# shehryar-malik/icrl

Measured on NVIDIA B200. Metric: learner transitions/sec per ICRL iteration at 1/2/4/8 B200 vs host CPU, higher is better.
Workload: dtype f32

## Files before the change

### icrl_b200/_lib.py

```python
import ctypes as C
import os

HERE = os.path.dirname(os.path.abspath(__file__))
LIB_PATH = os.path.join(HERE, "libicrl_b200.so")

ABI_VERSION = 2
MAX_SELECT, MAX_HIDDEN, CN_MAX_WIDTH = 512, 3, 64
PPO_STATS_PER_STEP = 8

c_float_p = C.POINTER(C.c_float)
c_void = C.c_void_p


class CnDesc(C.Structure):
    _fields_ = [
        ("obs_dim", C.c_int32), ("acs_dim", C.c_int32), ("is_discrete", C.c_int32), ("n_select", C.c_int32),
        ("select", C.c_int32 * MAX_SELECT), ("n_hidden", C.c_int32), ("hidden", C.c_int32 * MAX_HIDDEN),
        ("has_norm", C.c_int32), ("has_clip_obs", C.c_int32), ("has_clip_acs", C.c_int32), ("clip_obs", C.c_double),
        ("params", c_void), ("obs_mean", c_void), ("obs_rstd", c_void), ("acs_low", c_void), ("acs_high", c_void),
    ]


class CnTrainCfg(C.Structure):
    _fields_ = [
        ("iterations", C.c_int32), ("importance_sampling", C.c_int32), ("per_step_is", C.c_int32),
        ("train_gail_lambda", C.c_int32), ("eps", C.c_float), ("regularizer_coeff", C.c_float),
        ("target_kl_old_new", C.c_float), ("target_kl_new_old", C.c_float), ("lr", C.c_double),
        ("adam_beta1", C.c_double), ("adam_beta2", C.c_double), ("adam_eps", C.c_double),
        ("batch_size", C.c_int32), ("perm", c_void),
    ]

# ... 41 lines not shown

SIGNATURES = {
    "icrl_abi_version": (C.c_int, []),
    "icrl_last_error": (C.c_char_p, []),
    "icrl_launch_count": (C.c_int64, []),
    "icrl_device_info": (C.c_int, [C.POINTER(C.c_int32), C.POINTER(C.c_int32)]),
    "icrl_measure_peaks": (C.c_int, [C.POINTER(C.c_double), c_void]),
    "icrl_cn_param_count": (C.c_int64, [C.POINTER(CnDesc)]),
    "icrl_cn_forward": (C.c_int, [C.POINTER(CnDesc), c_void, C.c_int32, c_void, C.c_int64, c_void, C.c_int32, c_void]),
    "icrl_cn_forward_host": (C.c_int, [C.POINTER(CnDesc), c_void, C.c_int32, c_void, C.c_int64, c_void, C.c_int32,
                                       c_void]),
    "icrl_cn_train": (C.c_int, [C.POINTER(CnDesc), C.POINTER(CnTrainCfg), c_void, C.c_int32, c_void, C.c_int64, c_void,
                                C.c_int32, c_void, C.c_int32, c_void, C.c_int64, c_void, c_void, C.POINTER(C.c_int64),
                                C.POINTER(CnTrainMetrics), c_void]),
    "icrl_cn_dist_bytes": (C.c_int64, [C.POINTER(CnDesc), C.c_int32]),
    "icrl_cn_train_dist": (C.c_int, [C.POINTER(CnDesc), C.POINTER(CnTrainCfg), c_void, C.c_int32, c_void, C.c_int64, c_void,
                                     C.c_int32, c_void, C.c_int32, c_void, C.c_int64, c_void, c_void, C.POINTER(C.c_int64),
                                     C.POINTER(CnTrainMetrics), C.POINTER(CnDist), c_void]),
    "icrl_dual_gae": (C.c_int, [c_void] * 8 + [C.c_int32, C.c_int32] + [C.c_double] * 4 + [c_void] * 5),
    "icrl_dual_gae_host": (C.c_int, [c_void] * 8 + [C.c_int32, C.c_int32] + [C.c_double] * 4 + [c_void] * 5),
    "icrl_ppo_param_count": (C.c_int64, [C.POINTER(PpoCfg)]),
    "icrl_ppo_train": (C.c_int, [C.POINTER(PpoCfg), C.POINTER(PpoData), c_void, c_void, c_void, C.c_int64, c_void,
                                 c_void, c_void]),
    "icrl_ppo_train_dist": (C.c_int, [C.POINTER(PpoCfg), C.POINTER(PpoData), c_void, c_void, c_void, C.c_int64, c_void,
                                      c_void, C.POINTER(PpoDist), c_void]),
    "icrl_ppo_local_advsums": (C.c_int, [C.POINTER(PpoCfg), C.POINTER(PpoData), c_void, c_void]),
    "icrl_comm_alloc": (C.c_int, [C.c_int64, C.POINTER(c_void), C.c_char_p]),
    "icrl_comm_open": (C.c_int, [C.c_char_p, C.POINTER(c_void)]),
    "icrl_comm_close": (C.c_int, [c_void]),
    "icrl_comm_free": (C.c_int, [c_void]),
    "icrl_policy_forward": (C.c_int, [C.POINTER(PpoCfg), c_void, c_void, C.c_int64, c_void, c_void, c_void, c_void]),
    "icrl_dual_update": (C.c_int, [c_void, c_void, C.c_int64, C.c_double, C.c_double, C.c_int64, C.c_double, c_void]),
    "icrl_cost_normalize": (C.c_int, [c_void, c_void, c_void, C.c_int32, C.c_int32, C.c_double, C.c_double, C.c_double,
                                      C.c_int32, C.c_int32, c_void, c_void, c_void]),
}


class IcrlError(RuntimeError):
    pass


_lib = None


def lib():
    global _lib
# ... 32 lines not shown
```

### icrl_b200/csrc/k4_common.cuh

```cuda
#pragma once
#include <math.h>
#include <stdlib.h>

#include "common.cuh"

namespace icrl {

constexpr int H = 64;
constexpr int RB = 64;
constexpr int NTH = 256;
constexpr int AMAX = 16;
constexpr int WA_LD = 68;
constexpr int LDH = 68;
constexpr float LOG_SQRT_2PI = 0.91893853320467274178f;
constexpr float HALF_LOG_2PI_PLUS_HALF = 1.4189385332046727418f;

__host__ __device__ inline int ppo_kp(int D) { return (D + 7) / 8 * 8; }
__host__ __device__ inline int ppo_ldx(int D) {
    const int kp = (D + 15) / 16 * 16;
    int ld = kp / 32 * 32 + 4;
    if (ld < kp) ld += 32;
    return ld;
}

// ... 50 lines not shown
    }
    return o;
}

inline int ppo_make_args(const icrl_ppo_cfg* c, PpoArgs& a) {
    ICRL_CHECK_ARG(c != nullptr, "ppo cfg is NULL");
    ICRL_CHECK_ARG(c->obs_dim >= 1, "obs_dim must be >= 1");
    ICRL_CHECK_ARG(c->act_dim >= 1 && c->act_dim <= AMAX, "act_dim %d out of range (1..%d)", c->act_dim, AMAX);
    bool per_trunk = false;
    for (int t = 0; t < 3; ++t) per_trunk |= c->trunk_hidden[t][0] != 0 || c->trunk_hidden[t][1] != 0;
    if (per_trunk) {
        static const char* const names[3] = {"pi", "vf", "cvf"};
        for (int t = 0; t < 3; ++t)
            ICRL_CHECK_ARG(c->trunk_hidden[t][0] >= 1 && c->trunk_hidden[t][0] <= H && c->trunk_hidden[t][1] >= 1 &&
                               c->trunk_hidden[t][1] <= H,
                           "trunk_hidden[%d] (%s) = (%d, %d): both widths must be in 1..%d (two hidden layers per trunk)", t,
                           names[t], c->trunk_hidden[t][0], c->trunk_hidden[t][1], H);
    } else {
        ICRL_CHECK_ARG(c->hidden[0] >= 1 && c->hidden[0] <= H && c->hidden[1] >= 1 && c->hidden[1] <= H,
                       "policy hidden sizes (%d, %d) must be in 1..%d (two hidden layers per trunk)", c->hidden[0],
                       c->hidden[1], H);
    }
    a.D = c->obs_dim; a.DP = ppo_ldx(c->obs_dim); a.KP = ppo_kp(c->obs_dim); a.A = c->act_dim; a.is_discrete = c->is_discrete;
    for (int t = 0; t < 3; ++t) {
        a.h0[t] = per_trunk ? c->trunk_hidden[t][0] : c->hidden[0];
        a.h1[t] = per_trunk ? c->trunk_hidden[t][1] : c->hidden[1];
    }
    a.T = c->T; a.E = c->E; a.N = c->T * c->E;
    a.B = c->batch_size > 0 ? c->batch_size : a.N;
    if (a.B > a.N && a.N > 0) a.B = a.N;
    a.n_epochs = c->n_epochs;
    a.steps_per_epoch = a.N > 0 ? (a.N + a.B - 1) / a.B : 0;
    a.max_steps = c->max_steps;
    a.has_target_kl = c->has_target_kl; a.has_clip_vf_r = c->has_clip_vf_reward; a.has_clip_vf_c = c->has_clip_vf_cost;
    a.clip_range = c->clip_range; a.clip_vf_r = c->clip_range_reward_vf; a.clip_vf_c = c->clip_range_cost_vf;
    a.ent_coef = c->ent_coef; a.vf_coef_r = c->reward_vf_coef; a.vf_coef_c = c->cost_vf_coef;
    a.max_grad_norm = c->max_grad_norm; a.nu = c->nu; a.target_kl = c->target_kl;
    a.lr = c->lr; a.beta1 = c->adam_beta1; a.beta2 = c->adam_beta2; a.adam_eps = c->adam_eps;
    ppo_fill_offsets(a);
    return 0;
}

}
```

### icrl_b200/csrc/k4_ppo_lag.cu

```cuda
#include <type_traits>

#include "k4_common.cuh"

namespace icrl {

__device__ __forceinline__ uint32_t cluster_ctarank() {
    uint32_t r;
    asm volatile("mov.u32 %0, %%cluster_ctarank;" : "=r"(r));
    return r;
}
__device__ __forceinline__ uint32_t cluster_nctarank() {
    uint32_t r;
    asm volatile("mov.u32 %0, %%cluster_nctarank;" : "=r"(r));
    return r;
}
__device__ __forceinline__ void cluster_sync_all() {
    asm volatile("barrier.cluster.arrive.release.aligned;\n\tbarrier.cluster.wait.acquire.aligned;" ::: "memory");
}
__device__ __forceinline__ void st_remote_f32(float* local_ptr, uint32_t rank, float v) {
    uint32_t a = smem_u32(local_ptr), ra;
    asm volatile("mapa.shared::cluster.u32 %0, %1, %2;" : "=r"(ra) : "r"(a), "r"(rank));
    asm volatile("st.shared::cluster.f32 [%0], %1;" ::"r"(ra), "f"(v) : "memory");
}

// ... 1465 lines not shown
    for (int e = 0; e < n_epochs; ++e) {
        a.n_epochs = 1;
        a.epoch_base = e;
        a.perm = perm + (size_t)e * a.N;
        a.stats = stats + (size_t)e * spe * ICRL_PPO_STATS_PER_STEP;
        a.advsums = advsums ? advsums + (size_t)e * spe * 4 : nullptr;
        a.step_before = step_before + (long long)e * spe;
        a.flag_base = flag_base + (unsigned int)(e * spe);
        ppo_gather_kernel<<<ggrid, 256, 0, st>>>(a, xs, as, ss, (long long)a.N, n_alloc);
        ICRL_LAUNCH_CHECK();
        ppo_stats_kernel<<<spe, 128, 0, st>>>(ss, advstats, a.N, a.B, spe, a.beta1, a.beta2, a.lr, a.step_before, a.advsums);
        ICRL_LAUNCH_CHECK();
        ICRL_CUDA(cudaMemsetAsync(sync, 0, 64, st));
        const cudaError_t err = cudaLaunchKernelEx(&cfg, kern, a);
        if (err != cudaSuccess) {
            set_error("wide ppo_train_kernel launch failed: %s", cudaGetErrorString(err));
            return (int)err;
        }
        count_launch();
    }
    return 0;
}

}

extern "C" {

int64_t icrl_ppo_param_count(const icrl_ppo_cfg* cfg) {
    icrl::PpoArgs a = {};
    if (icrl::ppo_make_args(cfg, a)) return -1;
    return icrl::ppo_fill_offsets(a);
}

static void ppo_print_timing(unsigned long long* timing_dev, cudaStream_t st, double steps);

static int ppo_train_impl(const icrl_ppo_cfg* cfg, const icrl_ppo_data* data, float* params, float* adam_m, float* adam_v,
                          int64_t adam_step_before, float* step_stats, int32_t* result, const icrl_ppo_dist* dist,
                          void* stream) {
    icrl::PpoArgs a = {};
    int rc = icrl::ppo_make_args(cfg, a);
    if (rc) return rc;
    if (dist) {
        ICRL_CHECK_ARG(dist->world >= 1 && dist->world <= ICRL_PPO_MAX_RANKS && dist->rank >= 0 && dist->rank < dist->world,
                       "bad rank/world (%d/%d)", dist->rank, dist->world);
        a.rank = dist->rank; a.world = dist->world; a.flag_base = dist->flag_base; a.advsums = dist->advsums;
        for (int r = 0; r < dist->world; ++r) {
            ICRL_CHECK_ARG(dist->world == 1 || (dist->recv[r] && dist->flags[r]), "peer buffer %d is NULL", r);
            a.recv[r] = dist->recv[r]; a.flags[r] = dist->flags[r];
        }
        ICRL_CHECK_ARG(dist->world == 1 || dist->advsums, "data-parallel mode needs the all-reduced advsums table");
    }
    ICRL_CHECK_ARG(data && params && adam_m && adam_v && step_stats && result, "NULL pointer passed to icrl_ppo_train");
    ICRL_CHECK_ARG(a.N > 0 && a.n_epochs > 0, "empty rollout buffer or n_epochs <= 0");
    ICRL_CHECK_ARG(data->observations && data->actions && data->old_log_prob && data->reward_advantages &&
                       data->reward_returns && data->cost_advantages && data->cost_returns && data->perm,
                   "NULL rollout array");
    ICRL_CHECK_ARG((!a.has_clip_vf_r || data->old_reward_values) && (!a.has_clip_vf_c || data->old_cost_values),
                   "value clipping enabled but old values are NULL");
    a.obs = data->observations; a.act = data->actions; a.old_logp = data->old_log_prob;
    a.old_vr = data->old_reward_values ? data->old_reward_values : data->reward_returns;
    a.adv_r = data->reward_advantages; a.ret_r = data->reward_returns;
    a.old_vc = data->old_cost_values ? data->old_cost_values : data->cost_returns;
    a.adv_c = data->cost_advantages; a.ret_c = data->cost_returns;
    a.perm = data->perm;
    a.nu_dev = data->nu_device;
    a.params = params; a.adam_m = adam_m; a.adam_v = adam_v; a.stats = step_stats; a.result = result;
    a.step_before = adam_step_before;
    if (a.world < 1) { a.world = 1; a.rank = 0; }
    {
        const char* m = getenv("ICRL_PPO_DIST_MODE");
        a.dist_mode = m ? atoi(m) : 0;
    }
    cudaStream_t st = (cudaStream_t)stream;
    ICRL_CUDA(cudaMemsetAsync(result, 0, 4 * sizeof(int32_t), st));
    const int n_tiles = a.KP / 8;
    const int nt1 = (n_tiles + 1) / 2;
    if (nt1 > 8) {
        icrl::set_error("obs_dim %d too large for the PPO kernel (max 128)", a.D);
        return ICRL_EUNSUPPORTED;
    }
    static unsigned long long* timing_dev = nullptr;
    const bool want_timing = getenv("ICRL_PPO_TIMING") != nullptr;
    if (want_timing && !timing_dev) cudaMalloc(&timing_dev, 128 * sizeof(unsigned long long));
    a.timing = want_timing ? timing_dev : nullptr;
    auto print_timing = [&](double steps) { ppo_print_timing(timing_dev, st, steps); };
    bool wide = a.B >= icrl::WIDE_MIN_BATCH;
    if (const char* m = getenv("ICRL_PPO_WIDE")) wide = atoi(m) != 0;
    int n_clusters = 1;
    if (wide) {
        int cap = 0;
        if (nt1 <= 1) rc = icrl::wide_max_clusters<1>(a, st, &cap);
        else if (nt1 <= 2) rc = icrl::wide_max_clusters<2>(a, st, &cap);
        else if (nt1 <= 4) rc = icrl::wide_max_clusters<4>(a, st, &cap);
        else rc = icrl::wide_max_clusters<8>(a, st, &cap);
        if (rc) return rc;
        if (cap > icrl::WIDE_MAXCTA / icrl::NCTA) cap = icrl::WIDE_MAXCTA / icrl::NCTA;
        const int useful = (a.B + icrl::RB - 1) / icrl::RB;
        n_clusters = cap < useful ? cap : useful;
        if (const char* m = getenv("ICRL_PPO_WIDE_CLUSTERS")) {
            const int c = atoi(m);
            if (c > 0) n_clusters = c < cap ? c : cap;
        }
        const int nt1r = nt1 <= 1 ? 1 : nt1 <= 2 ? 2 : nt1 <= 4 ? 4 : 8;
        const int F = icrl::NTW2 * 4 + nt1r * 4 + 4 + 1 + 5;
        if (n_clusters < 1 || 2 * n_clusters * icrl::WIDE_SMAX < F) wide = false;
    }
    {
        const int epochs_alloc = wide ? 1 : a.n_epochs;
        const int total_steps = epochs_alloc * a.steps_per_epoch;
        const long long n_rows = (long long)epochs_alloc * a.N, n_alloc = n_rows + icrl::RB;
        const int aw = a.is_discrete ? 1 : a.A;
        a.AP = (aw + 3) / 4 * 4;
        void *xs, *as, *ss, *advstats;
        if ((rc = icrl::device_scratch(icrl::SLOT_PPO0, (size_t)n_alloc * a.DP * 4, &xs))) return rc;
        if ((rc = icrl::device_scratch(icrl::SLOT_PPO1, (size_t)total_steps * 8 * sizeof(float), &advstats))) return rc;
        if ((rc = icrl::device_scratch(icrl::SLOT_PPO2, (size_t)n_alloc * a.AP * 4, &as))) return rc;
        if ((rc = icrl::device_scratch(icrl::SLOT_PPO3, (size_t)n_alloc * 8 * 4, &ss))) return rc;
        if (wide) {
            if (nt1 <= 1) rc = icrl::launch_ppo_wide<1>(a, st, n_clusters, (float*)xs, (float*)as, (float*)ss, (float*)advstats);
            else if (nt1 <= 2) rc = icrl::launch_ppo_wide<2>(a, st, n_clusters, (float*)xs, (float*)as, (float*)ss, (float*)advstats);
            else if (nt1 <= 4) rc = icrl::launch_ppo_wide<4>(a, st, n_clusters, (float*)xs, (float*)as, (float*)ss, (float*)advstats);
            else rc = icrl::launch_ppo_wide<8>(a, st, n_clusters, (float*)xs, (float*)as, (float*)ss, (float*)advstats);
            if (rc == 0 && want_timing) {
                fprintf(stderr, "[ppo timing] many-cluster kernel, %d clusters, last epoch (%d steps of %d rows):\n", n_clusters,
                        a.steps_per_epoch, a.B);
                print_timing((double)a.steps_per_epoch);
            }
            return rc;
        }
        const long long blocks = (n_alloc + 7) / 8;
        const int grid = (int)(blocks < 8LL * icrl::sm_count() ? blocks : 8LL * icrl::sm_count());
        icrl::ppo_gather_kernel<<<grid, 256, 0, st>>>(a, (float*)xs, (float*)as, (float*)ss, n_rows, n_alloc);
        ICRL_LAUNCH_CHECK();
        icrl::ppo_stats_kernel<<<total_steps, 128, 0, st>>>((const float*)ss, (float*)advstats, a.N, a.B, a.steps_per_epoch,
                                                            a.beta1, a.beta2, a.lr, a.step_before, a.advsums);
        ICRL_LAUNCH_CHECK();
        a.xs = (const float*)xs; a.as = (const float*)as; a.ss = (const float*)ss;
        a.advstats = (const float*)advstats;
    }
    if (nt1 <= 1) rc = icrl::launch_ppo<1>(a, st);
    else if (nt1 <= 2) rc = icrl::launch_ppo<2>(a, st);
    else if (nt1 <= 4) rc = icrl::launch_ppo<4>(a, st);
    else rc = icrl::launch_ppo<8>(a, st);
    if (rc == 0 && want_timing) print_timing((double)(a.max_steps > 0 ? a.max_steps : a.n_epochs * a.steps_per_epoch));
    return rc;
}

static void ppo_print_timing(unsigned long long* timing_dev, cudaStream_t st, double steps) {
    unsigned long long h[128];
    cudaStreamSynchronize(st);
    cudaMemcpy(h, timing_dev, sizeof(h), cudaMemcpyDeviceToHost);
    const char* names[11] = {"wait+sync", "prefetch", "L1", "L2", "head", "headgrad+dH2", "dW2+dH1", "dW1", "blockreduce+stats",
                             "norm xchg", "adam"};
    for (int r = 0; r < icrl::NCTA; r += (r == 0 ? 1 : 2)) {
        const unsigned long long* t = h + r * 20;
        fprintf(stderr, "[ppo timing] cta %d cycles/step:", r);
        double tot = 0;
        for (int i = 0; i < 11; ++i) { fprintf(stderr, " %s=%.0f", names[i], t[i] / steps); tot += t[i] / steps; }
        for (int i = 11; i < 19; ++i) tot += t[i] / steps;
        fprintf(stderr, " | head: dot=%.0f logp=%.0f, headgrad: dHW=%.0f bias/logstd=%.0f dH2=%.0f | exchange: pair wait+add=%.0f "
                        "rank send=%.0f rank poll+sum=%.0f | total=%.0f\n",
                t[11] / steps, t[12] / steps, t[13] / steps, t[14] / steps, t[15] / steps, t[16] / steps, t[17] / steps,
                t[18] / steps, tot);
    }
}

int icrl_ppo_train(const icrl_ppo_cfg* cfg, const icrl_ppo_data* data, float* params, float* adam_m, float* adam_v,
                   int64_t adam_step_before, float* step_stats, int32_t* result, void* stream) {
    return ppo_train_impl(cfg, data, params, adam_m, adam_v, adam_step_before, step_stats, result, nullptr, stream);
}

int icrl_ppo_train_dist(const icrl_ppo_cfg* cfg, const icrl_ppo_data* data, float* params, float* adam_m, float* adam_v,
                        int64_t adam_step_before, float* step_stats, int32_t* result, const icrl_ppo_dist* dist,
                        void* stream) {
    ICRL_CHECK_ARG(dist != nullptr, "dist is NULL");
    return ppo_train_impl(cfg, data, params, adam_m, adam_v, adam_step_before, step_stats, result, dist, stream);
}

int icrl_ppo_local_advsums(const icrl_ppo_cfg* cfg, const icrl_ppo_data* data, double* advsums_out, void* stream) {
    icrl::PpoArgs a = {};
    int rc = icrl::ppo_make_args(cfg, a);
    if (rc) return rc;
    ICRL_CHECK_ARG(data && advsums_out && data->perm && data->reward_advantages && data->cost_advantages && a.N > 0,
                   "NULL pointer passed to icrl_ppo_local_advsums");
    icrl::ppo_local_advsums_kernel<<<a.n_epochs * a.steps_per_epoch, 128, 0, (cudaStream_t)stream>>>(
        data->perm, data->reward_advantages, data->cost_advantages, a.T, a.E, a.N, a.B, a.steps_per_epoch, advsums_out);
    ICRL_LAUNCH_CHECK();
    return 0;
}

}
```

### icrl_b200/learner.py

```python
import ctypes as C
from dataclasses import dataclass
from typing import Optional, Tuple

import numpy as np
import torch as th

from . import _lib
from .constraint_net import ConstraintNet
from .device import resolve_device
from .dual_variable import DualVariable
from .policies import ActorTwoCriticsPolicy
from .vec_env import RunningMeanStd
from .spaces import Box, Discrete


@dataclass
class Workload:
    name: str
    obs_dim: int
    act_dim: int
    is_discrete: bool
    cn_hidden: Tuple[int, ...]
    n_steps: int = 2048
    n_envs: int = 5
# ... 111 lines not shown
        self.costs = z(R, T, E)
        self.costs_norm = z(R, T, E) if w.normalize_cost else self.costs
        rms = RunningMeanStd(shape=())
        rms.update(np.zeros(E))
        self.cost_state = th.tensor([rms.mean, rms.var, rms.count] + [0.0] * E, dtype=th.float64, device=d)
        self.adv_r, self.ret_r, self.adv_c, self.ret_c = z(R, T, E), z(R, T, E), z(R, T, E), z(R, T, E)
        self.steps_per_epoch = (self.n + w.batch_size - 1) // w.batch_size
        self.stats = z(R, w.n_epochs * self.steps_per_epoch, _lib.PPO_STATS_PER_STEP)
        self.result = th.zeros(R, 4, dtype=th.int32, device=d)
        self.perm = th.empty(R, w.n_epochs, self.n, dtype=th.int32, device=d)
        if w.nominal_rows:
            self.nom_obs, self.nom_acs = th.from_numpy(no).to(d), th.from_numpy(
                na.reshape(-1) if w.is_discrete else na).to(d)
            self.exp_obs, self.exp_acs = th.from_numpy(eo).to(d), th.from_numpy(
                ea.reshape(-1) if w.is_discrete else ea).to(d)
            off = np.zeros(len(lengths) + 1, np.int32)
            off[1:] = np.cumsum(lengths)
            self.offsets, self.n_episodes = th.from_numpy(off).to(d), len(lengths)
        self.max_steps = 0
        if comm is not None and comm.world > 1:
            self.advsums = th.zeros(w.n_epochs * self.steps_per_epoch, 4, dtype=th.float64, device=d)
            self.cost_mean = th.zeros(1, device=d)
            self.shard_k2(seed)
        self.refresh_behaviour()
        self.new_permutations(seed)

    def refresh_behaviour(self):
        w = self.w
        for r in range(w.rollouts):
            obs = self.data["obs"][r].reshape(self.n, w.obs_dim)
            acts = self.data["actions"][r].reshape(self.n, -1)
            v, cv, lp, _ = self.policy.evaluate_actions(obs, acts.reshape(-1) if w.is_discrete else acts)
            self.reward_values[r] = v.reshape(w.n_steps, self.E)
            self.cost_values[r] = cv.reshape(w.n_steps, self.E)
            self.log_probs[r] = lp.reshape(w.n_steps, self.E)
            self.last_rv[r], self.last_cv[r] = self.reward_values[r, -1], self.cost_values[r, -1]

    def new_permutations(self, seed):
        rs = np.random.RandomState(seed)
        w = self.w
        perms = np.stack([np.stack([rs.permutation(self.n) for _ in range(w.n_epochs)]) for _ in range(w.rollouts)])
        self.perm.copy_(th.from_numpy(perms.astype(np.int32)))

    def ppo_cfg(self):
        w = self.w
        return self.policy.make_cfg(
            T=w.n_steps, E=self.E, batch_size=w.batch_size, n_epochs=w.n_epochs, has_target_kl=0, target_kl=0.0,
            clip_range=w.clip_range, ent_coef=0.0, reward_vf_coef=0.5, cost_vf_coef=0.5, max_grad_norm=0.5,
            nu=0.0, max_steps=self.max_steps)

    def run(self, stream=None):
        w, L = self.w, _lib.lib()
        st = _lib.current_stream()
        desc = self.cn._get_desc()
        cfg = self.ppo_cfg()
        pol = self.policy
        for r in range(w.rollouts):
            _lib.check(L.icrl_cn_forward(C.byref(desc), _lib.ptr(self.data["orig_obs"][r]), 0,
                                         _lib.ptr(self.data["actions"][r]), self.n, _lib.ptr(self.costs[r]), 0, st))
            if w.normalize_cost:
                _lib.check(L.icrl_cost_normalize(_lib.ptr(self.costs[r]), _lib.ptr(self.data["dones"][r]),
                                                 _lib.ptr(self.data["last_dones"][r]), w.n_steps, self.E, 0.99, 1e-8, 10.0,
                                                 1, 1, _lib.ptr(self.cost_state), _lib.ptr(self.costs_norm[r]), st))
            _lib.check(L.icrl_dual_gae(
                _lib.ptr(self.data["rewards"][r]), _lib.ptr(self.reward_values[r]), _lib.ptr(self.costs_norm[r]),
                _lib.ptr(self.cost_values[r]), _lib.ptr(self.data["dones"][r]), _lib.ptr(self.last_rv[r]),
                _lib.ptr(self.last_cv[r]), _lib.ptr(self.data["last_dones"][r]), w.n_steps, self.E, 0.99,
                w.reward_gae_lambda, 0.99, w.cost_gae_lambda, _lib.ptr(self.adv_r[r]), _lib.ptr(self.ret_r[r]),
                _lib.ptr(self.adv_c[r]), _lib.ptr(self.ret_c[r]), st))
            data = _lib.PpoData()
            data.nu_device = self.dual.nu.state[4:5].data_ptr()
            data.observations, data.actions = self.data["obs"][r].data_ptr(), self.data["actions"][r].data_ptr()
            data.old_log_prob = self.log_probs[r].data_ptr()
            data.old_reward_values, data.old_cost_values = self.reward_values[r].data_ptr(), self.cost_values[r].data_ptr()
            data.reward_advantages, data.reward_returns = self.adv_r[r].data_ptr(), self.ret_r[r].data_ptr()
            data.cost_advantages, data.cost_returns = self.adv_c[r].data_ptr(), self.ret_c[r].data_ptr()
            data.perm = self.perm[r].data_ptr()
            dp = self.comm is not None and self.comm.world > 1
            if not dp:
                _lib.check(L.icrl_ppo_train(C.byref(cfg), C.byref(data), _lib.ptr(pol._params), _lib.ptr(pol._adam_m),
                                            _lib.ptr(pol._adam_v), pol.optimizer.step_count, _lib.ptr(self.stats[r]),
                                            _lib.ptr(self.result[r]), st))
            else:
                _lib.check(L.icrl_ppo_local_advsums(C.byref(cfg), C.byref(data), _lib.ptr(self.advsums), st))
                self.comm.all_reduce_sum(self.advsums)
                desc_d = self.comm.descriptor(self.advsums)
                _lib.check(L.icrl_ppo_train_dist(C.byref(cfg), C.byref(data), _lib.ptr(pol._params), _lib.ptr(pol._adam_m),
                                                 _lib.ptr(pol._adam_v), pol.optimizer.step_count, _lib.ptr(self.stats[r]),
                                                 _lib.ptr(self.result[r]), C.byref(desc_d), _lib.current_stream()))
                self.comm.advance(self.steps_taken_per_rollout())
            pol.optimizer.step_count += self.steps_taken_per_rollout()
            if not dp:
                _lib.check(L.icrl_dual_update(_lib.ptr(self.dual.nu.state), _lib.ptr(self.costs[r]), self.n, 0.0,
                                              float(w.penalty_learning_rate), self.dual.steps, self.dual.nu.clamp_min(), st))
            else:
                self.cost_mean.copy_(self.costs[r].mean().reshape(1))
                self.comm.all_reduce_sum(self.cost_mean)
                self.cost_mean /= self.comm.world
                _lib.check(L.icrl_dual_update(_lib.ptr(self.dual.nu.state), _lib.ptr(self.cost_mean), 1, 0.0,
                                              float(w.penalty_learning_rate), self.dual.steps, self.dual.nu.clamp_min(),
                                              _lib.current_stream()))
            self.dual.steps += 1
        if w.backward_iters > 0 and w.nominal_rows > 0:
            self._cn_train_device()

    def check(self):
        res = self.result.cpu().numpy()
        if (res[:, 2] != 0).any():
            raise _lib.IcrlError(f"PPO kernel exchange time-out in rollouts {np.nonzero(res[:, 2])[0].tolist()}: the "
                                 "replicated parameters are no longer valid")
        want = self.steps_taken_per_rollout()
        if (res[:, 1] != want).any():
            raise _lib.IcrlError(f"PPO kernel took {res[:, 1].tolist()} optimiser steps, expected {want} per rollout")

    def steps_taken_per_rollout(self):
        full = self.w.n_epochs * self.steps_per_epoch
        return min(full, self.max_steps) if self.max_steps > 0 else full

    def _cn_train_device(self):
        w, cn = self.w, self.cn
        g = cn.optimizer.param_groups[0]
        cfg = _lib.CnTrainCfg(
            iterations=w.backward_iters, importance_sampling=1, per_step_is=int(w.per_step_is), train_gail_lambda=0,
            eps=float(cn.eps), regularizer_coeff=float(w.cn_reg), target_kl_old_new=float(cn.target_kl_old_new),
            target_kl_new_old=float(cn.target_kl_new_old), lr=float(g["lr"]), adam_beta1=0.9, adam_beta2=0.999,
            adam_eps=float(g["eps"]), batch_size=0, perm=None)
        metrics = _lib.CnTrainMetrics()
        step = C.c_int64(cn.optimizer.step_count)
        args = (C.byref(cn._get_desc()), C.byref(cfg), _lib.ptr(self.nom_obs), 0, _lib.ptr(self.nom_acs), w.nominal_rows,
                _lib.ptr(self.offsets), self.n_episodes, _lib.ptr(self.exp_obs), 0, _lib.ptr(self.exp_acs),
                self.exp_obs.shape[0], _lib.ptr(cn._adam_m), _lib.ptr(cn._adam_v), C.byref(step), C.byref(metrics))
        cc = getattr(cn, "comm", None)
        if cc is None or cc.world == 1:
            _lib.check(_lib.lib().icrl_cn_train(*args, _lib.current_stream()))
        else:
            d = cc.descriptor(w.nominal_rows * cc.world, self.exp_rows_global, self.n_episodes * cc.world,
                              self.n_episodes * cc.rank)
            _lib.check(_lib.lib().icrl_cn_train_dist(*args, C.byref(d), _lib.current_stream()))
            cc.advance(w.backward_iters)
        cn.optimizer.step_count = int(step.value)
        self.last_cn_metrics = metrics

    def shard_k2(self, seed: int):
        w, cn, comm = self.w, self.cn, self.comm
        if comm is None or comm.world == 1 or not w.nominal_rows:
            return
        cn.enable_data_parallel(max_episodes=max(1024, 2 * self.n_episodes * comm.world))
        _, _, no, na, _ = synth_demos(w, seed)
        self.nom_obs = th.from_numpy(no).to(self.dev)
        self.nom_acs = th.from_numpy(na.reshape(-1) if w.is_discrete else na).to(self.dev)
        n = self.exp_obs.shape[0]
        self.exp_rows_global = n
        lo, hi = n * comm.rank // comm.world, n * (comm.rank + 1) // comm.world
        self.exp_obs, self.exp_acs = self.exp_obs[lo:hi].contiguous(), self.exp_acs[lo:hi].contiguous()
```

### include/icrl_b200.h

```cpp
#ifndef ICRL_B200_H
#define ICRL_B200_H

#include <stdint.h>

#ifdef __cplusplus
extern "C" {
#endif

#define ICRL_ABI_VERSION 2

#define ICRL_EINVAL (-1)
#define ICRL_EUNSUPPORTED (-2)
#define ICRL_EPEER (-3)

#define ICRL_MAX_SELECT 512
#define ICRL_MAX_HIDDEN 3
#define ICRL_CN_MAX_WIDTH 64

int icrl_abi_version(void);
const char* icrl_last_error(void);
int64_t icrl_launch_count(void);
int icrl_device_info(int32_t* sm_count, int32_t* cc);
int icrl_measure_peaks(double* tflops2, void* stream);

// ... 97 lines not shown
    int32_t max_steps;
    int32_t trunk_hidden[3][2];
} icrl_ppo_cfg;

typedef struct icrl_ppo_data {
    const float* observations;
    const float* actions;
    const float* old_log_prob;
    const float* old_reward_values;
    const float* reward_advantages;
    const float* reward_returns;
    const float* old_cost_values;
    const float* cost_advantages;
    const float* cost_returns;
    const int32_t* perm;
    const float* nu_device;
} icrl_ppo_data;

#define ICRL_PPO_STATS_PER_STEP 8
int64_t icrl_ppo_param_count(const icrl_ppo_cfg* cfg);
int icrl_ppo_train(const icrl_ppo_cfg* cfg, const icrl_ppo_data* data, float* params, float* adam_m, float* adam_v,
                   int64_t adam_step_before, float* step_stats, int32_t* result, void* stream);


#define ICRL_PPO_MAX_RANKS 8
#define ICRL_PPO_RECV_BYTES (32 * 1024 * 1024)
#define ICRL_PPO_FLAG_BYTES (2 * ICRL_PPO_MAX_RANKS * 4 * 4)

int icrl_comm_alloc(int64_t bytes, void** dev_ptr, unsigned char* handle64);
int icrl_comm_open(const unsigned char* handle64, void** dev_ptr);
int icrl_comm_close(void* dev_ptr);
int icrl_comm_free(void* dev_ptr);

typedef struct icrl_ppo_dist {
    int32_t rank, world;
    float* recv[ICRL_PPO_MAX_RANKS];
    uint32_t* flags[ICRL_PPO_MAX_RANKS];
    uint32_t flag_base;
    const double* advsums;
} icrl_ppo_dist;

int icrl_ppo_local_advsums(const icrl_ppo_cfg* cfg, const icrl_ppo_data* data, double* advsums_out, void* stream);
int icrl_ppo_train_dist(const icrl_ppo_cfg* cfg, const icrl_ppo_data* data, float* params, float* adam_m, float* adam_v,
                        int64_t adam_step_before, float* step_stats, int32_t* result, const icrl_ppo_dist* dist,
                        void* stream);

// ... 15 lines not shown
```

Before: 763,500.

## Pipeline PPO staging and cost relabel on side stream with double-buffered stages

```diff
diff --git a/icrl_b200/_lib.py b/icrl_b200/_lib.py
--- a/icrl_b200/_lib.py
+++ b/icrl_b200/_lib.py
@@ -7,6 +7,7 @@
 ABI_VERSION = 2
 MAX_SELECT, MAX_HIDDEN, CN_MAX_WIDTH = 512, 3, 64
 PPO_STATS_PER_STEP = 8
+PPO_WIDE_MIN_BATCH = 2048
 
 c_float_p = C.POINTER(C.c_float)
 c_void = C.c_void_p
@@ -94,6 +95,10 @@
     "icrl_ppo_param_count": (C.c_int64, [C.POINTER(PpoCfg)]),
     "icrl_ppo_train": (C.c_int, [C.POINTER(PpoCfg), C.POINTER(PpoData), c_void, c_void, c_void, C.c_int64, c_void,
                                  c_void, c_void]),
+    "icrl_ppo_stage_bytes": (C.c_int64, [C.POINTER(PpoCfg)]),
+    "icrl_ppo_prepare": (C.c_int, [C.POINTER(PpoCfg), C.POINTER(PpoData), C.c_int64, c_void, C.c_int64, c_void]),
+    "icrl_ppo_train_staged": (C.c_int, [C.POINTER(PpoCfg), C.POINTER(PpoData), c_void, c_void, c_void, c_void, C.c_int64,
+                                        c_void, c_void, c_void]),
     "icrl_ppo_train_dist": (C.c_int, [C.POINTER(PpoCfg), C.POINTER(PpoData), c_void, c_void, c_void, C.c_int64, c_void,
                                       c_void, C.POINTER(PpoDist), c_void]),
     "icrl_ppo_local_advsums": (C.c_int, [C.POINTER(PpoCfg), C.POINTER(PpoData), c_void, c_void]),
diff --git a/icrl_b200/csrc/k4_common.cuh b/icrl_b200/csrc/k4_common.cuh
--- a/icrl_b200/csrc/k4_common.cuh
+++ b/icrl_b200/csrc/k4_common.cuh
@@ -96,6 +96,7 @@
                        c->hidden[1], H);
     }
     a.D = c->obs_dim; a.DP = ppo_ldx(c->obs_dim); a.KP = ppo_kp(c->obs_dim); a.A = c->act_dim; a.is_discrete = c->is_discrete;
+    a.AP = ((c->is_discrete ? 1 : c->act_dim) + 3) / 4 * 4;
     for (int t = 0; t < 3; ++t) {
         a.h0[t] = per_trunk ? c->trunk_hidden[t][0] : c->hidden[0];
         a.h1[t] = per_trunk ? c->trunk_hidden[t][1] : c->hidden[1];
diff --git a/icrl_b200/csrc/k4_ppo_lag.cu b/icrl_b200/csrc/k4_ppo_lag.cu
--- a/icrl_b200/csrc/k4_ppo_lag.cu
+++ b/icrl_b200/csrc/k4_ppo_lag.cu
@@ -1511,6 +1511,74 @@
     return 0;
 }
 
+static int ppo_pick_regime(const PpoArgs& a, int nt1, cudaStream_t st, int* n_clusters) {
+    *n_clusters = 0;
+    bool wide = a.B >= WIDE_MIN_BATCH;
+    if (const char* m = getenv("ICRL_PPO_WIDE")) wide = atoi(m) != 0;
+    if (!wide) return 0;
+    int cap = 0, rc;
+    if (nt1 <= 1) rc = wide_max_clusters<1>(a, st, &cap);
+    else if (nt1 <= 2) rc = wide_max_clusters<2>(a, st, &cap);
+    else if (nt1 <= 4) rc = wide_max_clusters<4>(a, st, &cap);
+    else rc = wide_max_clusters<8>(a, st, &cap);
+    if (rc) return rc;
+    if (cap > WIDE_MAXCTA / NCTA) cap = WIDE_MAXCTA / NCTA;
+    const int useful = (a.B + RB - 1) / RB;
+    int n = cap < useful ? cap : useful;
+    if (const char* m = getenv("ICRL_PPO_WIDE_CLUSTERS")) {
+        const int c = atoi(m);
+        if (c > 0) n = c < cap ? c : cap;
+    }
+    const int nt1r = nt1 <= 1 ? 1 : nt1 <= 2 ? 2 : nt1 <= 4 ? 4 : 8;
+    const int F = NTW2 * 4 + nt1r * 4 + 4 + 1 + 5;
+    if (n < 1 || 2 * n * WIDE_SMAX < F) return 0;
+    *n_clusters = n;
+    return 0;
+}
+
+struct PpoStage {
+    size_t xs, as, ss, advstats, bytes;
+    long long n_rows, n_alloc;
+    int total_steps;
+};
+inline size_t align16(size_t b) { return (b + 15) & ~(size_t)15; }
+static PpoStage ppo_stage_layout(const PpoArgs& a) {
+    PpoStage s;
+    s.total_steps = a.n_epochs * a.steps_per_epoch;
+    s.n_rows = (long long)a.n_epochs * a.N;
+    s.n_alloc = s.n_rows + RB;
+    s.xs = 0;
+    s.as = align16(s.xs + (size_t)s.n_alloc * a.DP * 4);
+    s.ss = align16(s.as + (size_t)s.n_alloc * a.AP * 4);
+    s.advstats = align16(s.ss + (size_t)s.n_alloc * 8 * 4);
+    s.bytes = align16(s.advstats + (size_t)s.total_steps * 8 * 4);
+    return s;
+}
+
+static int ppo_prepare_stage(const PpoArgs& a, const PpoStage& L, void* stage, cudaStream_t st) {
+    char* base = (char*)stage;
+    float *xs = (float*)(base + L.xs), *as = (float*)(base + L.as), *ss = (float*)(base + L.ss);
+    const long long blocks = (L.n_alloc + 7) / 8;
+    const int grid = (int)(blocks < 8LL * sm_count() ? blocks : 8LL * sm_count());
+    ppo_gather_kernel<<<grid, 256, 0, st>>>(a, xs, as, ss, L.n_rows, L.n_alloc);
+    ICRL_LAUNCH_CHECK();
+    ppo_stats_kernel<<<L.total_steps, 128, 0, st>>>(ss, (float*)(base + L.advstats), a.N, a.B, a.steps_per_epoch, a.beta1,
+                                                    a.beta2, a.lr, a.step_before, a.advsums);
+    ICRL_LAUNCH_CHECK();
+    return 0;
+}
+
+static int ppo_train_stage(PpoArgs a, const PpoStage& L, const void* stage, int nt1, cudaStream_t st) {
+    const char* base = (const char*)stage;
+    a.xs = (const float*)(base + L.xs); a.as = (const float*)(base + L.as); a.ss = (const float*)(base + L.ss);
+    a.advstats = (const float*)(base + L.advstats);
+    ICRL_CUDA(cudaMemsetAsync(a.result, 0, 4 * sizeof(int32_t), st));
+    if (nt1 <= 1) return launch_ppo<1>(a, st);
+    if (nt1 <= 2) return launch_ppo<2>(a, st);
+    if (nt1 <= 4) return launch_ppo<4>(a, st);
+    return launch_ppo<8>(a, st);
+}
+
 }
 
 extern "C" {
@@ -1522,6 +1590,53 @@
 }
 
 static void ppo_print_timing(unsigned long long* timing_dev, cudaStream_t st, double steps);
+
+static unsigned long long* ppo_timing_buffer() {
+    static unsigned long long* timing_dev = nullptr;
+    if (getenv("ICRL_PPO_TIMING") == nullptr) return nullptr;
+    if (!timing_dev) cudaMalloc(&timing_dev, 128 * sizeof(unsigned long long));
+    return timing_dev;
+}
+
+static int ppo_nt1(const icrl::PpoArgs& a, int* nt1) {
+    *nt1 = (a.KP / 8 + 1) / 2;
+    if (*nt1 > 8) {
+        icrl::set_error("obs_dim %d too large for the PPO kernel (max 128)", a.D);
+        return ICRL_EUNSUPPORTED;
+    }
+    return 0;
+}
+
+static int ppo_bind_rollout(icrl::PpoArgs& a, const icrl_ppo_data* data) {
+    ICRL_CHECK_ARG(data, "NULL icrl_ppo_data");
+    ICRL_CHECK_ARG(a.N > 0 && a.n_epochs > 0, "empty rollout buffer or n_epochs <= 0");
+    ICRL_CHECK_ARG(data->observations && data->actions && data->old_log_prob && data->reward_advantages &&
+                       data->reward_returns && data->cost_advantages && data->cost_returns && data->perm,
+                   "NULL rollout array");
+    ICRL_CHECK_ARG((!a.has_clip_vf_r || data->old_reward_values) && (!a.has_clip_vf_c || data->old_cost_values),
+                   "value clipping enabled but old values are NULL");
+    a.obs = data->observations; a.act = data->actions; a.old_logp = data->old_log_prob;
+    a.old_vr = data->old_reward_values ? data->old_reward_values : data->reward_returns;
+    a.adv_r = data->reward_advantages; a.ret_r = data->reward_returns;
+    a.old_vc = data->old_cost_values ? data->old_cost_values : data->cost_returns;
+    a.adv_c = data->cost_advantages; a.ret_c = data->cost_returns;
+    a.perm = data->perm;
+    return 0;
+}
+
+static int ppo_bind_train(icrl::PpoArgs& a, const icrl_ppo_data* data, float* params, float* adam_m, float* adam_v,
+                          int64_t adam_step_before, float* step_stats, int32_t* result) {
+    ICRL_CHECK_ARG(data && params && adam_m && adam_v && step_stats && result, "NULL pointer passed to icrl_ppo_train");
+    ICRL_CHECK_ARG(a.N > 0 && a.n_epochs > 0, "empty rollout buffer or n_epochs <= 0");
+    a.nu_dev = data->nu_device;
+    a.params = params; a.adam_m = adam_m; a.adam_v = adam_v; a.stats = step_stats; a.result = result;
+    a.step_before = adam_step_before;
+    if (a.world < 1) { a.world = 1; a.rank = 0; }
+    const char* m = getenv("ICRL_PPO_DIST_MODE");
+    a.dist_mode = m ? atoi(m) : 0;
+    a.timing = ppo_timing_buffer();
+    return 0;
+}
 
 static int ppo_train_impl(const icrl_ppo_cfg* cfg, const icrl_ppo_data* data, float* params, float* adam_m, float* adam_v,
                           int64_t adam_step_before, float* step_stats, int32_t* result, const icrl_ppo_dist* dist,
@@ -1539,100 +1654,58 @@
         }
         ICRL_CHECK_ARG(dist->world == 1 || dist->advsums, "data-parallel mode needs the all-reduced advsums table");
     }
-    ICRL_CHECK_ARG(data && params && adam_m && adam_v && step_stats && result, "NULL pointer passed to icrl_ppo_train");
+    if ((rc = ppo_bind_train(a, data, params, adam_m, adam_v, adam_step_before, step_stats, result))) return rc;
+    if ((rc = ppo_bind_rollout(a, data))) return rc;
+    cudaStream_t st = (cudaStream_t)stream;
+    int nt1, n_clusters;
+    if ((rc = ppo_nt1(a, &nt1))) return rc;
+    if ((rc = icrl::ppo_pick_regime(a, nt1, st, &n_clusters))) return rc;
+    if (n_clusters == 0) {
+        const icrl::PpoStage L = icrl::ppo_stage_layout(a);
+        void* stage;
+        if ((rc = icrl::device_scratch(icrl::SLOT_PPO0, L.bytes, &stage))) return rc;
+        if ((rc = icrl::ppo_prepare_stage(a, L, stage, st))) return rc;
+        rc = icrl::ppo_train_stage(a, L, stage, nt1, st);
+        if (rc == 0 && a.timing)
+            ppo_print_timing(a.timing, st, (double)(a.max_steps > 0 ? a.max_steps : a.n_epochs * a.steps_per_epoch));
+        return rc;
+    }
+    ICRL_CUDA(cudaMemsetAsync(result, 0, 4 * sizeof(int32_t), st));
+    const long long n_alloc = (long long)a.N + icrl::RB;
+    void *xs, *as, *ss, *advstats;
+    if ((rc = icrl::device_scratch(icrl::SLOT_PPO0, (size_t)n_alloc * a.DP * 4, &xs))) return rc;
+    if ((rc = icrl::device_scratch(icrl::SLOT_PPO1, (size_t)a.steps_per_epoch * 8 * sizeof(float), &advstats))) return rc;
+    if ((rc = icrl::device_scratch(icrl::SLOT_PPO2, (size_t)n_alloc * a.AP * 4, &as))) return rc;
+    if ((rc = icrl::device_scratch(icrl::SLOT_PPO3, (size_t)n_alloc * 8 * 4, &ss))) return rc;
+    if (nt1 <= 1) rc = icrl::launch_ppo_wide<1>(a, st, n_clusters, (float*)xs, (float*)as, (float*)ss, (float*)advstats);
+    else if (nt1 <= 2) rc = icrl::launch_ppo_wide<2>(a, st, n_clusters, (float*)xs, (float*)as, (float*)ss, (float*)advstats);
+    else if (nt1 <= 4) rc = icrl::launch_ppo_wide<4>(a, st, n_clusters, (float*)xs, (float*)as, (float*)ss, (float*)advstats);
+    else rc = icrl::launch_ppo_wide<8>(a, st, n_clusters, (float*)xs, (float*)as, (float*)ss, (float*)advstats);
+    if (rc == 0 && a.timing) {
+        fprintf(stderr, "[ppo timing] many-cluster kernel, %d clusters, last epoch (%d steps of %d rows):\n", n_clusters,
+                a.steps_per_epoch, a.B);
+        ppo_print_timing(a.timing, st, (double)a.steps_per_epoch);
+    }
+    return rc;
+}
+
+static int ppo_staged_args(const icrl_ppo_cfg* cfg, const void* stage, cudaStream_t st, icrl::PpoArgs& a, int* nt1,
+                           icrl::PpoStage* L) {
+    int rc = icrl::ppo_make_args(cfg, a);
+    if (rc) return rc;
     ICRL_CHECK_ARG(a.N > 0 && a.n_epochs > 0, "empty rollout buffer or n_epochs <= 0");
-    ICRL_CHECK_ARG(data->observations && data->actions && data->old_log_prob && data->reward_advantages &&
-                       data->reward_returns && data->cost_advantages && data->cost_returns && data->perm,
-                   "NULL rollout array");
-    ICRL_CHECK_ARG((!a.has_clip_vf_r || data->old_reward_values) && (!a.has_clip_vf_c || data->old_cost_values),
-                   "value clipping enabled but old values are NULL");
-    a.obs = data->observations; a.act = data->actions; a.old_logp = data->old_log_prob;
-    a.old_vr = data->old_reward_values ? data->old_reward_values : data->reward_returns;
-    a.adv_r = data->reward_advantages; a.ret_r = data->reward_returns;
-    a.old_vc = data->old_cost_values ? data->old_cost_values : data->cost_returns;
-    a.adv_c = data->cost_advantages; a.ret_c = data->cost_returns;
-    a.perm = data->perm;
-    a.nu_dev = data->nu_device;
-    a.params = params; a.adam_m = adam_m; a.adam_v = adam_v; a.stats = step_stats; a.result = result;
-    a.step_before = adam_step_before;
-    if (a.world < 1) { a.world = 1; a.rank = 0; }
-    {
-        const char* m = getenv("ICRL_PPO_DIST_MODE");
-        a.dist_mode = m ? atoi(m) : 0;
-    }
-    cudaStream_t st = (cudaStream_t)stream;
-    ICRL_CUDA(cudaMemsetAsync(result, 0, 4 * sizeof(int32_t), st));
-    const int n_tiles = a.KP / 8;
-    const int nt1 = (n_tiles + 1) / 2;
-    if (nt1 > 8) {
-        icrl::set_error("obs_dim %d too large for the PPO kernel (max 128)", a.D);
+    ICRL_CHECK_ARG(stage != nullptr, "NULL stage passed to icrl_ppo_prepare / icrl_ppo_train_staged");
+    ICRL_CHECK_ARG(((uintptr_t)stage & 15u) == 0, "stage %p is not 16-byte aligned", stage);
+    if ((rc = ppo_nt1(a, nt1))) return rc;
+    int n_clusters;
+    if ((rc = icrl::ppo_pick_regime(a, *nt1, st, &n_clusters))) return rc;
+    if (n_clusters != 0) {
+        icrl::set_error("batch_size %d runs on the many-cluster kernel (%d clusters), which stages one epoch per launch: use "
+                        "icrl_ppo_train", a.B, n_clusters);
         return ICRL_EUNSUPPORTED;
     }
-    static unsigned long long* timing_dev = nullptr;
-    const bool want_timing = getenv("ICRL_PPO_TIMING") != nullptr;
-    if (want_timing && !timing_dev) cudaMalloc(&timing_dev, 128 * sizeof(unsigned long long));
-    a.timing = want_timing ? timing_dev : nullptr;
-    auto print_timing = [&](double steps) { ppo_print_timing(timing_dev, st, steps); };
-    bool wide = a.B >= icrl::WIDE_MIN_BATCH;
-    if (const char* m = getenv("ICRL_PPO_WIDE")) wide = atoi(m) != 0;
-    int n_clusters = 1;
-    if (wide) {
-        int cap = 0;
-        if (nt1 <= 1) rc = icrl::wide_max_clusters<1>(a, st, &cap);
-        else if (nt1 <= 2) rc = icrl::wide_max_clusters<2>(a, st, &cap);
-        else if (nt1 <= 4) rc = icrl::wide_max_clusters<4>(a, st, &cap);
-        else rc = icrl::wide_max_clusters<8>(a, st, &cap);
-        if (rc) return rc;
-        if (cap > icrl::WIDE_MAXCTA / icrl::NCTA) cap = icrl::WIDE_MAXCTA / icrl::NCTA;
-        const int useful = (a.B + icrl::RB - 1) / icrl::RB;
-        n_clusters = cap < useful ? cap : useful;
-        if (const char* m = getenv("ICRL_PPO_WIDE_CLUSTERS")) {
-            const int c = atoi(m);
-            if (c > 0) n_clusters = c < cap ? c : cap;
-        }
-        const int nt1r = nt1 <= 1 ? 1 : nt1 <= 2 ? 2 : nt1 <= 4 ? 4 : 8;
-        const int F = icrl::NTW2 * 4 + nt1r * 4 + 4 + 1 + 5;
-        if (n_clusters < 1 || 2 * n_clusters * icrl::WIDE_SMAX < F) wide = false;
-    }
-    {
-        const int epochs_alloc = wide ? 1 : a.n_epochs;
-        const int total_steps = epochs_alloc * a.steps_per_epoch;
-        const long long n_rows = (long long)epochs_alloc * a.N, n_alloc = n_rows + icrl::RB;
-        const int aw = a.is_discrete ? 1 : a.A;
-        a.AP = (aw + 3) / 4 * 4;
-        void *xs, *as, *ss, *advstats;
-        if ((rc = icrl::device_scratch(icrl::SLOT_PPO0, (size_t)n_alloc * a.DP * 4, &xs))) return rc;
-        if ((rc = icrl::device_scratch(icrl::SLOT_PPO1, (size_t)total_steps * 8 * sizeof(float), &advstats))) return rc;
-        if ((rc = icrl::device_scratch(icrl::SLOT_PPO2, (size_t)n_alloc * a.AP * 4, &as))) return rc;
-        if ((rc = icrl::device_scratch(icrl::SLOT_PPO3, (size_t)n_alloc * 8 * 4, &ss))) return rc;
-        if (wide) {
-            if (nt1 <= 1) rc = icrl::launch_ppo_wide<1>(a, st, n_clusters, (float*)xs, (float*)as, (float*)ss, (float*)advstats);
-            else if (nt1 <= 2) rc = icrl::launch_ppo_wide<2>(a, st, n_clusters, (float*)xs, (float*)as, (float*)ss, (float*)advstats);
-            else if (nt1 <= 4) rc = icrl::launch_ppo_wide<4>(a, st, n_clusters, (float*)xs, (float*)as, (float*)ss, (float*)advstats);
-            else rc = icrl::launch_ppo_wide<8>(a, st, n_clusters, (float*)xs, (float*)as, (float*)ss, (float*)advstats);
-            if (rc == 0 && want_timing) {
-                fprintf(stderr, "[ppo timing] many-cluster kernel, %d clusters, last epoch (%d steps of %d rows):\n", n_clusters,
-                        a.steps_per_epoch, a.B);
-                print_timing((double)a.steps_per_epoch);
-            }
-            return rc;
-        }
-        const long long blocks = (n_alloc + 7) / 8;
-        const int grid = (int)(blocks < 8LL * icrl::sm_count() ? blocks : 8LL * icrl::sm_count());
-        icrl::ppo_gather_kernel<<<grid, 256, 0, st>>>(a, (float*)xs, (float*)as, (float*)ss, n_rows, n_alloc);
-        ICRL_LAUNCH_CHECK();
-        icrl::ppo_stats_kernel<<<total_steps, 128, 0, st>>>((const float*)ss, (float*)advstats, a.N, a.B, a.steps_per_epoch,
-                                                            a.beta1, a.beta2, a.lr, a.step_before, a.advsums);
-        ICRL_LAUNCH_CHECK();
-        a.xs = (const float*)xs; a.as = (const float*)as; a.ss = (const float*)ss;
-        a.advstats = (const float*)advstats;
-    }
-    if (nt1 <= 1) rc = icrl::launch_ppo<1>(a, st);
-    else if (nt1 <= 2) rc = icrl::launch_ppo<2>(a, st);
-    else if (nt1 <= 4) rc = icrl::launch_ppo<4>(a, st);
-    else rc = icrl::launch_ppo<8>(a, st);
-    if (rc == 0 && want_timing) print_timing((double)(a.max_steps > 0 ? a.max_steps : a.n_epochs * a.steps_per_epoch));
-    return rc;
+    *L = icrl::ppo_stage_layout(a);
+    return 0;
 }
 
 static void ppo_print_timing(unsigned long long* timing_dev, cudaStream_t st, double steps) {
@@ -1659,6 +1732,45 @@
     return ppo_train_impl(cfg, data, params, adam_m, adam_v, adam_step_before, step_stats, result, nullptr, stream);
 }
 
+int64_t icrl_ppo_stage_bytes(const icrl_ppo_cfg* cfg) {
+    icrl::PpoArgs a = {};
+    if (icrl::ppo_make_args(cfg, a)) return -1;
+    if (a.N <= 0 || a.n_epochs <= 0) {
+        icrl::set_error("empty rollout buffer or n_epochs <= 0");
+        return -1;
+    }
+    return (int64_t)icrl::ppo_stage_layout(a).bytes;
+}
+
+int icrl_ppo_prepare(const icrl_ppo_cfg* cfg, const icrl_ppo_data* data, int64_t adam_step_before, void* stage,
+                     int64_t stage_bytes, void* stream) {
+    icrl::PpoArgs a = {};
+    icrl::PpoStage L;
+    int nt1, rc;
+    cudaStream_t st = (cudaStream_t)stream;
+    if ((rc = ppo_staged_args(cfg, stage, st, a, &nt1, &L))) return rc;
+    ICRL_CHECK_ARG(stage_bytes >= (int64_t)L.bytes, "stage of %lld bytes is too small (%lld needed: icrl_ppo_stage_bytes)",
+                   (long long)stage_bytes, (long long)L.bytes);
+    if ((rc = ppo_bind_rollout(a, data))) return rc;
+    a.step_before = adam_step_before;
+    return icrl::ppo_prepare_stage(a, L, stage, st);
+}
+
+int icrl_ppo_train_staged(const icrl_ppo_cfg* cfg, const icrl_ppo_data* data, const void* stage, float* params,
+                          float* adam_m, float* adam_v, int64_t adam_step_before, float* step_stats, int32_t* result,
+                          void* stream) {
+    icrl::PpoArgs a = {};
+    icrl::PpoStage L;
+    int nt1, rc;
+    cudaStream_t st = (cudaStream_t)stream;
+    if ((rc = ppo_staged_args(cfg, stage, st, a, &nt1, &L))) return rc;
+    if ((rc = ppo_bind_train(a, data, params, adam_m, adam_v, adam_step_before, step_stats, result))) return rc;
+    rc = icrl::ppo_train_stage(a, L, stage, nt1, st);
+    if (rc == 0 && a.timing)
+        ppo_print_timing(a.timing, st, (double)(a.max_steps > 0 ? a.max_steps : a.n_epochs * a.steps_per_epoch));
+    return rc;
+}
+
 int icrl_ppo_train_dist(const icrl_ppo_cfg* cfg, const icrl_ppo_data* data, float* params, float* adam_m, float* adam_v,
                         int64_t adam_step_before, float* step_stats, int32_t* result, const icrl_ppo_dist* dist,
                         void* stream) {
diff --git a/icrl_b200/learner.py b/icrl_b200/learner.py
--- a/icrl_b200/learner.py
+++ b/icrl_b200/learner.py
@@ -157,6 +157,16 @@
             self.advsums = th.zeros(w.n_epochs * self.steps_per_epoch, 4, dtype=th.float64, device=d)
             self.cost_mean = th.zeros(1, device=d)
             self.shard_k2(seed)
+        self.pipelined = (comm is None or comm.world == 1) and min(w.batch_size, self.n) < _lib.PPO_WIDE_MIN_BATCH
+        if self.pipelined:
+            self.side = th.cuda.Stream(device=d)
+            nb = _lib.lib().icrl_ppo_stage_bytes(C.byref(self.ppo_cfg()))
+            if nb < 0:
+                _lib.check(-1)
+            self.stages = [th.empty(nb, dtype=th.uint8, device=d) for _ in range(2)]
+            self.ready = [th.cuda.Event() for _ in range(R)]
+            self.consumed = [th.cuda.Event() for _ in range(R)]
+            self.entry, self.side_done = th.cuda.Event(), th.cuda.Event()
         self.refresh_behaviour()
         self.new_permutations(seed)
 
@@ -185,33 +195,94 @@
             nu=0.0, max_steps=self.max_steps)
 
     def run(self, stream=None):
+        if self.pipelined:
+            self._run_pipelined()
+        else:
+            self._run_serial()
+
+    def _relabel_and_gae(self, r, desc, st):
+        w, L = self.w, _lib.lib()
+        _lib.check(L.icrl_cn_forward(C.byref(desc), _lib.ptr(self.data["orig_obs"][r]), 0,
+                                     _lib.ptr(self.data["actions"][r]), self.n, _lib.ptr(self.costs[r]), 0, st))
+        if w.normalize_cost:
+            _lib.check(L.icrl_cost_normalize(_lib.ptr(self.costs[r]), _lib.ptr(self.data["dones"][r]),
+                                             _lib.ptr(self.data["last_dones"][r]), w.n_steps, self.E, 0.99, 1e-8, 10.0,
+                                             1, 1, _lib.ptr(self.cost_state), _lib.ptr(self.costs_norm[r]), st))
+        _lib.check(L.icrl_dual_gae(
+            _lib.ptr(self.data["rewards"][r]), _lib.ptr(self.reward_values[r]), _lib.ptr(self.costs_norm[r]),
+            _lib.ptr(self.cost_values[r]), _lib.ptr(self.data["dones"][r]), _lib.ptr(self.last_rv[r]),
+            _lib.ptr(self.last_cv[r]), _lib.ptr(self.data["last_dones"][r]), w.n_steps, self.E, 0.99,
+            w.reward_gae_lambda, 0.99, w.cost_gae_lambda, _lib.ptr(self.adv_r[r]), _lib.ptr(self.ret_r[r]),
+            _lib.ptr(self.adv_c[r]), _lib.ptr(self.ret_c[r]), st))
+
+    def _ppo_data(self, r):
+        data = _lib.PpoData()
+        data.nu_device = self.dual.nu.state[4:5].data_ptr()
+        data.observations, data.actions = self.data["obs"][r].data_ptr(), self.data["actions"][r].data_ptr()
+        data.old_log_prob = self.log_probs[r].data_ptr()
+        data.old_reward_values, data.old_cost_values = self.reward_values[r].data_ptr(), self.cost_values[r].data_ptr()
+        data.reward_advantages, data.reward_returns = self.adv_r[r].data_ptr(), self.ret_r[r].data_ptr()
+        data.cost_advantages, data.cost_returns = self.adv_c[r].data_ptr(), self.ret_c[r].data_ptr()
+        data.perm = self.perm[r].data_ptr()
+        return data
+
+    def _dual_step(self, r, st):
+        w = self.w
+        _lib.check(_lib.lib().icrl_dual_update(_lib.ptr(self.dual.nu.state), _lib.ptr(self.costs[r]), self.n, 0.0,
+                                               float(w.penalty_learning_rate), self.dual.steps, self.dual.nu.clamp_min(),
+                                               st))
+        self.dual.steps += 1
+
+    def _run_pipelined(self):
+        w, L = self.w, _lib.lib()
+        R = w.rollouts
+        main, side = th.cuda.current_stream(), self.side
+        st_main, st_side = C.c_void_p(main.cuda_stream), C.c_void_p(side.cuda_stream)
+        desc = self.cn._get_desc()
+        cfg = self.ppo_cfg()
+        pol = self.policy
+        per_rollout = self.steps_taken_per_rollout()
+        step0 = pol.optimizer.step_count
+        stage_bytes = self.stages[0].numel()
+        data = [self._ppo_data(r) for r in range(R)]
+
+        def prepare(r):
+            if r >= 2:
+                side.wait_event(self.consumed[r - 2])
+            self._relabel_and_gae(r, desc, st_side)
+            _lib.check(L.icrl_ppo_prepare(C.byref(cfg), C.byref(data[r]), step0 + r * per_rollout,
+                                          _lib.ptr(self.stages[r % 2]), stage_bytes, st_side))
+            self.ready[r].record(side)
+
+        self.entry.record(main)
+        side.wait_event(self.entry)
+        prepare(0)
+        for r in range(R):
+            main.wait_event(self.ready[r])
+            _lib.check(L.icrl_ppo_train_staged(C.byref(cfg), C.byref(data[r]), _lib.ptr(self.stages[r % 2]),
+                                               _lib.ptr(pol._params), _lib.ptr(pol._adam_m), _lib.ptr(pol._adam_v),
+                                               step0 + r * per_rollout, _lib.ptr(self.stats[r]),
+                                               _lib.ptr(self.result[r]), st_main))
+            if r + 1 < R:
+                prepare(r + 1)
+            elif w.backward_iters > 0 and w.nominal_rows > 0:
+                self._cn_train_device(st_side)
+            self.consumed[r].record(main)
+            self._dual_step(r, st_main)
+        pol.optimizer.step_count = step0 + R * per_rollout
+        self.side_done.record(side)
+        main.wait_event(self.side_done)
+
+    def _run_serial(self):
         w, L = self.w, _lib.lib()
         st = _lib.current_stream()
         desc = self.cn._get_desc()
         cfg = self.ppo_cfg()
         pol = self.policy
+        dp = self.comm is not None and self.comm.world > 1
         for r in range(w.rollouts):
-            _lib.check(L.icrl_cn_forward(C.byref(desc), _lib.ptr(self.data["orig_obs"][r]), 0,
-                                         _lib.ptr(self.data["actions"][r]), self.n, _lib.ptr(self.costs[r]), 0, st))
-            if w.normalize_cost:
-                _lib.check(L.icrl_cost_normalize(_lib.ptr(self.costs[r]), _lib.ptr(self.data["dones"][r]),
-                                                 _lib.ptr(self.data["last_dones"][r]), w.n_steps, self.E, 0.99, 1e-8, 10.0,
-                                                 1, 1, _lib.ptr(self.cost_state), _lib.ptr(self.costs_norm[r]), st))
-            _lib.check(L.icrl_dual_gae(
-                _lib.ptr(self.data["rewards"][r]), _lib.ptr(self.reward_values[r]), _lib.ptr(self.costs_norm[r]),
-                _lib.ptr(self.cost_values[r]), _lib.ptr(self.data["dones"][r]), _lib.ptr(self.last_rv[r]),
-                _lib.ptr(self.last_cv[r]), _lib.ptr(self.data["last_dones"][r]), w.n_steps, self.E, 0.99,
-                w.reward_gae_lambda, 0.99, w.cost_gae_lambda, _lib.ptr(self.adv_r[r]), _lib.ptr(self.ret_r[r]),
-                _lib.ptr(self.adv_c[r]), _lib.ptr(self.ret_c[r]), st))
-            data = _lib.PpoData()
-            data.nu_device = self.dual.nu.state[4:5].data_ptr()
-            data.observations, data.actions = self.data["obs"][r].data_ptr(), self.data["actions"][r].data_ptr()
-            data.old_log_prob = self.log_probs[r].data_ptr()
-            data.old_reward_values, data.old_cost_values = self.reward_values[r].data_ptr(), self.cost_values[r].data_ptr()
-            data.reward_advantages, data.reward_returns = self.adv_r[r].data_ptr(), self.ret_r[r].data_ptr()
-            data.cost_advantages, data.cost_returns = self.adv_c[r].data_ptr(), self.ret_c[r].data_ptr()
-            data.perm = self.perm[r].data_ptr()
-            dp = self.comm is not None and self.comm.world > 1
+            self._relabel_and_gae(r, desc, st)
+            data = self._ppo_data(r)
             if not dp:
                 _lib.check(L.icrl_ppo_train(C.byref(cfg), C.byref(data), _lib.ptr(pol._params), _lib.ptr(pol._adam_m),
                                             _lib.ptr(pol._adam_v), pol.optimizer.step_count, _lib.ptr(self.stats[r]),
@@ -226,8 +297,7 @@
                 self.comm.advance(self.steps_taken_per_rollout())
             pol.optimizer.step_count += self.steps_taken_per_rollout()
             if not dp:
-                _lib.check(L.icrl_dual_update(_lib.ptr(self.dual.nu.state), _lib.ptr(self.costs[r]), self.n, 0.0,
-                                              float(w.penalty_learning_rate), self.dual.steps, self.dual.nu.clamp_min(), st))
+                self._dual_step(r, st)
             else:
                 self.cost_mean.copy_(self.costs[r].mean().reshape(1))
                 self.comm.all_reduce_sum(self.cost_mean)
@@ -235,9 +305,9 @@
                 _lib.check(L.icrl_dual_update(_lib.ptr(self.dual.nu.state), _lib.ptr(self.cost_mean), 1, 0.0,
                                               float(w.penalty_learning_rate), self.dual.steps, self.dual.nu.clamp_min(),
                                               _lib.current_stream()))
-            self.dual.steps += 1
+                self.dual.steps += 1
         if w.backward_iters > 0 and w.nominal_rows > 0:
-            self._cn_train_device()
+            self._cn_train_device(_lib.current_stream())
 
     def check(self):
         res = self.result.cpu().numpy()
@@ -252,7 +322,7 @@
         full = self.w.n_epochs * self.steps_per_epoch
         return min(full, self.max_steps) if self.max_steps > 0 else full
 
-    def _cn_train_device(self):
+    def _cn_train_device(self, st):
         w, cn = self.w, self.cn
         g = cn.optimizer.param_groups[0]
         cfg = _lib.CnTrainCfg(
@@ -267,11 +337,11 @@
                 self.exp_obs.shape[0], _lib.ptr(cn._adam_m), _lib.ptr(cn._adam_v), C.byref(step), C.byref(metrics))
         cc = getattr(cn, "comm", None)
         if cc is None or cc.world == 1:
-            _lib.check(_lib.lib().icrl_cn_train(*args, _lib.current_stream()))
+            _lib.check(_lib.lib().icrl_cn_train(*args, st))
         else:
             d = cc.descriptor(w.nominal_rows * cc.world, self.exp_rows_global, self.n_episodes * cc.world,
                               self.n_episodes * cc.rank)
-            _lib.check(_lib.lib().icrl_cn_train_dist(*args, C.byref(d), _lib.current_stream()))
+            _lib.check(_lib.lib().icrl_cn_train_dist(*args, C.byref(d), st))
             cc.advance(w.backward_iters)
         cn.optimizer.step_count = int(step.value)
         self.last_cn_metrics = metrics
diff --git a/include/icrl_b200.h b/include/icrl_b200.h
--- a/include/icrl_b200.h
+++ b/include/icrl_b200.h
@@ -143,6 +143,13 @@
 int icrl_ppo_train(const icrl_ppo_cfg* cfg, const icrl_ppo_data* data, float* params, float* adam_m, float* adam_v,
                    int64_t adam_step_before, float* step_stats, int32_t* result, void* stream);
 
+int64_t icrl_ppo_stage_bytes(const icrl_ppo_cfg* cfg);
+int icrl_ppo_prepare(const icrl_ppo_cfg* cfg, const icrl_ppo_data* data, int64_t adam_step_before, void* stage,
+                     int64_t stage_bytes, void* stream);
+int icrl_ppo_train_staged(const icrl_ppo_cfg* cfg, const icrl_ppo_data* data, const void* stage, float* params,
+                          float* adam_m, float* adam_v, int64_t adam_step_before, float* step_stats, int32_t* result,
+                          void* stream);
+
 
 #define ICRL_PPO_MAX_RANKS 8
 #define ICRL_PPO_RECV_BYTES (32 * 1024 * 1024)
```

Result: faster. 782,300 (median of 6 runs) (+2.5%).
